# WestlyPark/StyleRenderer

Hardware: AMD Instinct MI355X
Metric: generator fwd+bwd images/sec at 256^2 (higher is better)
Workload: dtype f32

## Files before the change

include/stylerenderer_amd.h:

```cpp
#ifndef STYLERENDERER_AMD_H_
#define STYLERENDERER_AMD_H_

#include <stddef.h>
#include <stdint.h>

#ifdef __cplusplus
extern "C" {
#endif

typedef void* sr_stream_t;

#define SR_OK 0
#define SR_EINVAL (-1)
#define SR_ERANGE (-2)

const char* sr_error_string(int code);
int sr_abi_version(void);

int sr_fused_bias_act(float* y, const float* x, const float* b, const float* ref, int act, int grad,
                      float alpha, float scale, int64_t size_x, int64_t step_b, int64_t size_b,
                      int use_bias, int use_ref, sr_stream_t stream);

int64_t sr_fused_act_bwd_scratch_floats(int64_t n, int64_t c, int64_t inner);
int sr_fused_act_bwd(float* gx, float* gb, const float* gy, const float* out, float alpha,
// ... 246 lines not shown
#define SR_CONV_PATH_S2_BF16 2
#define SR_CONV_PATH_S2_WINO 3
#define SR_CONV_PATH_GEMM1X1 4
#define SR_CONV_PATH_CONVT_TAPS 5
#define SR_CONV_PATH_CONVT_BF16 6
#define SR_CONV_PATH_CONVT_FUSED_KS 7
#define SR_CONV_PATH_CONVT_FUSED 8
#define SR_CONV_PATH_CONVT_WINO 9
#define SR_CONV_PATH_STRIPS 0x100
int sr_conv2d_path(int64_t B, int64_t C, int64_t N, int64_t IH, int64_t IW, int64_t OH, int64_t OW, int ksize, int stride,
                   int pad, int transposed, const float* in, const float* out, const float* wt, int64_t wt_ld,
                   int have_scratch);
int64_t sr_conv2d_path_floats(int64_t B, int64_t C, int64_t N, int64_t IH, int64_t IW, int64_t OH, int64_t OW, int ksize,
                              int stride, int pad, int transposed, const float* in, const float* out, const float* wt,
                              int64_t wt_ld, int have_scratch);

int sr_conv2d_generic(float* y, const float* x, const float* w, const float* bias, int64_t B, int64_t C, int64_t N,
                      int64_t IH, int64_t IW, int64_t OH, int64_t OW, int kh, int kw, int sy, int sx, int py, int px,
                      sr_stream_t stream);
int sr_conv2d_generic_dgrad(float* dx, const float* g, const float* w, int64_t B, int64_t C, int64_t N, int64_t IH,
                            int64_t IW, int64_t OH, int64_t OW, int kh, int kw, int sy, int sx, int py, int px,
                            sr_stream_t stream);
int sr_conv2d_generic_wgrad(float* dw, const float* x, const float* g, int64_t B, int64_t C, int64_t N, int64_t IH,
                            int64_t IW, int64_t OH, int64_t OW, int kh, int kw, int sy, int sx, int py, int px,
                            sr_stream_t stream);
int sr_conv2d_mfma_ex(float* out, const float* in, const float* wt, const float* iscale,
                      const float* oscale, const float* obias, int64_t B, int64_t C, int64_t N,
                      int64_t wt_ld, int64_t IH, int64_t IW, int64_t OH, int64_t OW, int ksize,
                      int stride, int pad, int transposed, int flags, float* scratch, sr_stream_t stream);
int sr_conv1x1_add_supported(int64_t B, int64_t C, int64_t N, int64_t wt_ld, int64_t P, const float* in, const float* wt,
                             const float* out, const float* addend);
int sr_conv1x1_add(float* out, const float* in, const float* wt, const float* oscale, const float* addend, int64_t B,
                   int64_t C, int64_t N, int64_t wt_ld, int64_t P, sr_stream_t stream);
int sr_conv2d_nba_ex(float* out, const float* in, const float* wt, const float* iscale, const float* oscale,
                     const float* noise, const float* noise_w, const float* abias, float alpha, float gain,
                     int64_t B, int64_t C, int64_t N, int64_t wt_ld, int64_t H, int64_t W, int64_t noise_bstride,
                     int flags, float* scratch, sr_stream_t stream);

int64_t sr_conv2d_wgrad_scratch_floats(int64_t B, int64_t C, int64_t N, int64_t IH, int64_t IW,
                                       int64_t OH, int64_t OW, int ksize, int stride, int pad,
                                       int transposed);
int sr_conv2d_wgrad_mfma(float* dwt, const float* x, const float* gy, const float* xscale,
                         const float* gscale, int64_t B, int64_t C, int64_t N, int64_t IH,
                         int64_t IW, int64_t OH, int64_t OW, int ksize, int stride, int pad,
                         int transposed, float* scratch, sr_stream_t stream);
#define SR_WGRAD_PATH_INVALID (-1)
#define SR_WGRAD_PATH_DIRECT 0
#define SR_WGRAD_PATH_SMALL3 1
#define SR_WGRAD_PATH_WINO 2
#define SR_WGRAD_PATH_BF16_1X1 3
#define SR_WGRAD_PATH_BF16_S2 4
#define SR_WGRAD_PATH_S2_DMA 5
#define SR_WGRAD_PATH_S2_WINO 6
int sr_conv2d_wgrad_path(int64_t B, int64_t C, int64_t N, int64_t IH, int64_t IW, int64_t OH, int64_t OW, int ksize,
                         int stride, int pad, int transposed, const float* x, const float* gy);
int64_t sr_conv2d_wgrad_path_floats(int64_t B, int64_t C, int64_t N, int64_t IH, int64_t IW, int64_t OH, int64_t OW,
                                    int ksize, int stride, int pad, int transposed, const float* x, const float* gy);
int64_t sr_conv2d_wgrad_style_floats(int64_t B, int64_t C, int64_t N, int64_t IH, int64_t IW, int64_t OH, int64_t OW,
                                     int ksize, int stride, int pad, int transposed, const float* x, const float* gy);
int sr_conv2d_wgrad_style(float* dwt, float* gis, const float* x, const float* gy, const float* iscale,
                          const float* gscale, const float* wt, int64_t ldw, int64_t B, int64_t C, int64_t N, int64_t IH,
                          int64_t IW, int64_t OH, int64_t OW, int ksize, int stride, int pad, int transposed,
                          float* scratch, float* part, sr_stream_t stream);

int sr_signal_bump(uint32_t* counter, sr_stream_t stream);
int sr_signal_set(uint32_t* word, const uint32_t* epoch, sr_stream_t stream);
// ... 150 lines not shown
```

stylerenderer_amd/_lib.py:

```python
import ctypes
import os

_HERE = os.path.dirname(os.path.abspath(__file__))
LIB_PATH = os.environ.get("STYLERENDERER_AMD_LIB") or os.path.join(_HERE, "libstylerenderer_hip.so")

_i = ctypes.c_int
_l = ctypes.c_int64
_f = ctypes.c_float
_d = ctypes.c_double
_p = ctypes.c_void_p

SIGNATURES = {
    "sr_error_string": (ctypes.c_char_p, [_i]),
    "sr_abi_version": (_i, []),
    "sr_fused_bias_act": (_i, [_p, _p, _p, _p, _i, _i, _f, _f, _l, _l, _l, _i, _i, _p]),
    "sr_fused_act_bwd_scratch_floats": (_l, [_l, _l, _l]),
    "sr_fused_act_bwd": (_i, [_p, _p, _p, _p, _f, _f, _l, _l, _l, _p, _p]),
    "sr_noise_bias_act": (_i, [_p] * 6 + [_f, _f] + [_l] * 4 + [_p]),
    "sr_noise_bias_act_bwd_scratch_floats": (_l, [_l, _l, _l]),
    "sr_noise_bias_act_bwd": (_i, [_p] * 6 + [_f, _f] + [_l] * 4 + [_p, _p]),
    "sr_noise_bias_act_bwd_dot_scratch_floats": (_l, [_l, _l, _l]),
    "sr_noise_bias_act_bwd_dot": (_i, [_p] * 9 + [_f, _f] + [_l] * 4 + [_p, _p]),
    "sr_conv2d_nba": (_i, [_p] * 8 + [_f, _f] + [_l] * 7 + [_p, _p]),
    "sr_conv2d_nba_ex": (_i, [_p] * 8 + [_f, _f] + [_l] * 7 + [_i, _p, _p]),
# ... 64 lines not shown
    "sr_conv2d_generic_dgrad": (_i, [_p] * 3 + [_l] * 7 + [_i] * 6 + [_p]),
    "sr_conv2d_generic_wgrad": (_i, [_p] * 3 + [_l] * 7 + [_i] * 6 + [_p]),
    "sr_blur_nba_bwd_scratch_floats": (_l, [_l, _l, _i, _i]),
    "sr_blur_nba_bwd": (_i, [_p] * 10 + [_f, _f, _l, _l] + [_i] * 5 + [_l, _p, _p]),
    "sr_rasterize_scratch_bytes": (_l, [_l, _l, _l, _l, _i]),
    "sr_rasterize_grad_state_ints": (_l, [_l, _l]),
    "sr_rasterize_forward_f32": (_i, [_l] * 5 + [_i] * 3 + [_p] * 5 + [_f, _p, _l, _p, _p, _p, _p, _p]),
    "sr_rasterize_levels_supported": (_i, [_i, _l, _l, _p, _p]),
    "sr_rasterize_forward_levels_f32": (_i, [_i, _l, _l, _l, _p, _p, _i, _i, _i, _p, _p, _f, _p, _l, _p, _p, _p, _p, _p]),
    "sr_rasterize_grad_levels_f32": (_i, [_i, _l, _l, _l, _p, _p, _i, _i, _p, _p, _l] + [_p] * 6 + [_l, _l] + [_p] * 3 + [_f, _p, _p]),
    "sr_rasterize_forward_f64": (_i, [_l] * 5 + [_i] * 3 + [_p] * 5 + [_d, _p, _l, _p, _p, _p, _p, _p]),
    "sr_rasterize_grad_scratch_bytes": (_l, [_l, _l, _l, _i]),
    "sr_rasterize_forward_cpu_f32": (_i, [_l] * 5 + [_i] * 3 + [_p] * 5 + [_f]),
    "sr_rasterize_forward_cpu_f64": (_i, [_l] * 5 + [_i] * 3 + [_p] * 5 + [_d]),
    "sr_rasterize_backward_cpu_f32": (_i, [_l] * 4 + [_i] + [_p] * 3 + [_f]),
    "sr_rasterize_backward_cpu_f64": (_i, [_l] * 4 + [_i] + [_p] * 3 + [_d]),
    "sr_rasterize_backward_f32": (_i, [_l] * 4 + [_i] * 2 + [_p] * 3 + [_f, _p]),
    "sr_rasterize_backward_f64": (_i, [_l] * 4 + [_i] * 2 + [_p] * 3 + [_d, _p]),
    "sr_rasterize_grad_f32": (_i, [_l] * 5 + [_i] * 2 + [_p, _p, _l] + [_p] * 6 + [_l, _l, _p, _p, _p, _f, _p, _p]),
    "sr_conv2d_wgrad_scratch_floats": (_l, [_l] * 7 + [_i] * 4),
    "sr_conv2d_wgrad_mfma": (_i, [_p] * 5 + [_l] * 7 + [_i] * 4 + [_p, _p]),
    "sr_conv2d_scratch_floats": (_l, [_l] * 7 + [_i] * 4),
    "sr_conv2d_mfma": (_i, [_p] * 6 + [_l] * 8 + [_i] * 4 + [_p, _p]),
    "sr_conv2d_uses_winograd": (_i, [_l] * 5 + [_p, _p]),
    "sr_conv2d_path": (_i, [_l] * 7 + [_i] * 4 + [_p, _p, _p, _l, _i]),
    "sr_conv2d_path_floats": (_l, [_l] * 7 + [_i] * 4 + [_p, _p, _p, _l, _i]),
    "sr_conv2d_wgrad_path": (_i, [_l] * 7 + [_i] * 4 + [_p, _p]),
    "sr_conv2d_wgrad_path_floats": (_l, [_l] * 7 + [_i] * 4 + [_p, _p]),
    "sr_conv2d_wgrad_style_floats": (_l, [_l] * 7 + [_i] * 4 + [_p, _p]),
    "sr_conv2d_wgrad_style": (_i, [_p] * 7 + [_l] * 8 + [_i] * 4 + [_p, _p, _p]),
    "sr_conv2d_mfma_ex": (_i, [_p] * 6 + [_l] * 8 + [_i] * 5 + [_p, _p]),
    "sr_conv1x1_add_supported": (_i, [_l] * 5 + [_p] * 4),
    "sr_conv1x1_add": (_i, [_p] * 5 + [_l] * 5 + [_p]),
    "sr_rasterize_grad_f64": (_i, [_l] * 5 + [_i] * 2 + [_p, _p, _l] + [_p] * 6 + [_l, _l, _p, _p, _p, _d, _p, _p]),
    "sr_pose_fwd": (_i, [_p, _p, _p, _p]),
    "sr_pose_bwd": (_i, [_p, _p, _p, _p, _p]),
    "sr_pose_batch_fwd": (_i, [_p, _p, _p, _l, _p]),
    "sr_affine3_fwd": (_i, [_p, _p, _p, _p, _l, _l, _l, _p]),
    "sr_affine3_bwd": (_i, [_p, _p, _p, _p, _l, _l, _l, _p]),
    "sr_morph_fwd": (_i, [_p] * 9 + [_f, _l, _l, _l, _p]),
    "sr_vertex_normals_bwd_f32": (_i, [_p] * 11 + [_l, _l, _l, _f, _p]),
    "sr_morph_gcoeff_scratch_floats": (_l, [_l, _l, _l]),
    "sr_morph_gcoeff": (_i, [_p] * 6 + [_f, _p, _l, _l, _l, _p]),
    "sr_morph_pose_bwd": (_i, [_p] * 5 + [_l, _p]),
    "sr_skin_joints_fwd": (_i, [_p] * 11 + [_f] + [_l] * 4 + [_p]),
    "sr_skin_fwd": (_i, [_p] * 7 + [_l] * 4 + [_p]),
    "sr_skin_bwd_scratch_floats": (_l, [_l, _l, _l]),
    "sr_skin_bwd": (_i, [_p] * 7 + [_l] * 3 + [_p]),
    "sr_skin_joints_bwd": (_i, [_p] * 11 + [_f, _p] + [_l] * 5 + [_p]),
    "sr_blend_z_floats": (_l, [_l, _l, _l]),
    "sr_blend_head": (_i, [_p] * 6 + [_f] + [_l] * 3 + [_p]),
    "sr_blend_fwd": (_i, [_p] * 8 + [_l] * 4 + [_p]),
    "sr_blend_gz": (_i, [_p] * 3 + [_l] * 4 + [_p]),
    "sr_blend_tail": (_i, [_p] * 5 + [_f, _p] + [_l] * 3 + [_p]),
    "sr_resample_u8_scratch_bytes": (_l, [_l] * 6 + [ctypes.POINTER(ctypes.c_int32)] + [_l] * 4),
    "sr_resample_u8": (_i, [_p, _p] + [_l] * 6 + [_p, _p, ctypes.POINTER(ctypes.c_int32), _l] * 2 + [_l] * 4
                       + [_i, _i, _p, _p]),
    "sr_warp_affine_u8": (_i, [_p, _p, _p] + [_l] * 7 + [_i, _i, _i, _p]),
    "sr_landmark_loss_fwd": (_i, [_p] * 8 + [_l] * 5 + [_f, _f, _p]),
    "sr_landmark_loss_bwd": (_i, [_p, _p, _p, _l, _p, _p, _p] + [_l] * 5 + [_i, _p]),
    "sr_landmark_dyn_fwd": (_i, [_p] * 15 + [_l] * 6 + [_i, _f, _f, _l, _l, _f, _f, _p]),
    "sr_landmark_dyn_bwd": (_i, [_p, _p, _p, _l] + [_p] * 7 + [_l] * 6 + [_i, _p]),
    "sr_region_fill": (_i, [_p, _p, _p] + [_l] * 6 + [_p]),
    "sr_region_grow": (_i, [_p, _p, _l, _l, _l, _i, _p]),
    "sr_region_blend_fwd": (_i, [_p] * 6 + [_l] * 4 + [_f] + [_l] * 4 + [_p]),
    "sr_region_blend_bwd": (_i, [_p] * 3 + [_l] * 4 + [_p]),
# ... 85 lines not shown
```

stylerenderer_amd/build.py:

```python
import os
import subprocess
import sys

HERE = os.path.dirname(os.path.abspath(__file__))
CSRC = os.path.join(HERE, "csrc")
LIB = os.path.join(HERE, "libstylerenderer_hip.so")
OBJ = os.path.join(HERE, "csrc", "_obj")

ARCH = "gfx950"
COMMON = ["--offload-arch=" + ARCH, "-O3", "-std=c++17", "-fPIC", "-Wno-unused-result",
          "-fhip-fp32-correctly-rounded-divide-sqrt"]
EXACT = ["-ffp-contract=off"]
NOSLP = ["-fno-slp-vectorize"]

SOURCES = [
    ("capi.hip", EXACT),
    ("fused_bias_act.hip", EXACT),
    ("upfirdn2d.hip", EXACT + NOSLP),
    ("rasterize.hip", EXACT),
    ("rasterize_keys.hip", EXACT),
    ("rasterize_tiled.hip", EXACT),
    ("rasterize_grad.hip", EXACT),
    ("fused_elem.hip", EXACT),
    ("weight_prep.hip", EXACT),
# ... 3 lines not shown
    ("landmark.hip", EXACT),
    ("region.hip", EXACT),
    ("texture.hip", EXACT),
    ("texture_sample.hip", EXACT),
    ("texture_mip.hip", EXACT),
    ("share.hip", EXACT),
    ("camera.hip", EXACT),
    ("light.hip", EXACT),
    ("morph.hip", []),
    ("skin.hip", []),
    ("blend.hip", []),
    ("lpips.hip", EXACT),
    ("ppl.hip", EXACT),
    ("augment.hip", EXACT),
    ("resample.hip", EXACT),
    ("warp.hip", EXACT),
    ("conv_dispatch.hip", []),
    ("conv_mfma.hip", []),
    ("convt_fused.hip", []),
    ("conv_wino.hip", []),
    ("conv_wgrad_wino.hip", []),
    ("conv_wgrad_dispatch.hip", []),
    ("conv_wgrad_mfma.hip", []),
    ("conv_wgrad_s2_dma.hip", []),
    ("conv_wgrad_small3.hip", []),
    ("conv_wgrad_reduce.hip", []),
    ("conv_wgrad_bf16x3.hip", []),
    ("conv_wgrad_s2_wino.hip", []),
    ("conv_s2_bf16x3.hip", []),
    ("conv_s2_wino.hip", []),
    ("convt_wino.hip", []),
    ("conv_generic.hip", []),
    ("conv1x1_gemm.hip", []),
    ("inception.hip", []),
]


def _hipcc():
    for c in (os.environ.get("HIPCC"), "/opt/rocm/bin/hipcc", "hipcc"):
        if c and (os.path.isabs(c) and os.path.exists(c) or not os.path.isabs(c)):
            return c
    return "hipcc"


def _deps(src):
    deps = [src, os.path.join(CSRC, "common.h"),
            os.path.join(HERE, "..", "include", "stylerenderer_amd.h"), os.path.abspath(__file__)]
    deps += [os.path.join(CSRC, f) for f in os.listdir(CSRC) if f.endswith(".h")]
    return max(os.path.getmtime(d) for d in deps if os.path.exists(d))


def build_library(force=False, verbose=False):
    os.makedirs(OBJ, exist_ok=True)
    hipcc = _hipcc()
    objs, rebuilt = [], False
    procs = []
    for name, extra in SOURCES:
        src = os.path.join(CSRC, name)
        obj = os.path.join(OBJ, name.replace(".hip", ".o"))
        objs.append(obj)
        if force or not os.path.exists(obj) or os.path.getmtime(obj) < _deps(src):
            cmd = [hipcc] + COMMON + extra + ["-c", src, "-o", obj]
            if verbose:
                print(" ".join(cmd))
            procs.append((name, subprocess.Popen(cmd, stdout=subprocess.PIPE, stderr=subprocess.STDOUT)))
            rebuilt = True
# ... 18 lines not shown
```

stylerenderer_amd/csrc/conv_mfma.hip:

```cpp
#include "conv_mfma.h"

#include "conv1x1_gemm.h"
#include "mfma_tile.h"

#include <algorithm>
#include <cstdlib>

namespace {

constexpr int BN = 128;
constexpr int BM = 128;

__device__ __attribute__((aligned(16))) const float g_zero_line[4] = {0.f, 0.f, 0.f, 0.f};
__device__ __attribute__((aligned(16))) const float g_ones_line[4] = {1.f, 1.f, 1.f, 1.f};

template <int IS, int TY, int TX, int PW, int PH, int PB, bool V4, bool TAP9 = false>
struct Geo {
    static constexpr bool ROT = V4 && IS == 2;
    static constexpr int NT = TY * TX;
    static constexpr int KC = NT >= 9 ? 4 : (NT >= 4 ? 8 : 16);
    static constexpr int EH = (PH - 1) * IS + TY;
    static constexpr int EW = (PW - 1) * IS + TX;
    static constexpr int LEAD = (V4 && !ROT) ? (TAP9 ? 4 : (TX > 1 ? 3 : 0)) : 0;
    static constexpr int EWP = ROT ? (EW + 3 + 3) / 4 * 4
                                   : (V4 ? (LEAD + EW + 3) / 4 * 4 : EW + ((EW % 2 == 0) ? 1 : 0));
    static constexpr int PLANE = PB * EH * EWP;
    static constexpr int W_FLOATS = NT * KC * BN;
    static constexpr int W_INSTR = W_FLOATS / 256;
    static constexpr int IMG_INSTR = V4 ? (KC * PLANE + 255) / 256 : 0;
    static constexpr int ST_INSTR = V4 ? (KC * PB + 63) / 64 : 0;
    static constexpr int IN_FLOATS = KC * PLANE + KC * PB;
    static constexpr int IN_INSTR = V4 ? IMG_INSTR + ST_INSTR : (IN_FLOATS + 63) / 64;
    static constexpr int S_BASE = V4 ? W_FLOATS + IMG_INSTR * 256 : W_FLOATS + KC * PLANE;
    static constexpr int BUF = V4 ? S_BASE + ST_INSTR * 64 : W_FLOATS + IN_INSTR * 64;
    static constexpr int W_PER_WAVE = (W_INSTR + 3) / 4;
// ... 521 lines not shown
    p.GH = p.IH + 1; p.GW = p.IW + 1;
    p.gy_base = p.gx_base = 0;
    p.osy = p.osx = 2; p.ooy = p.oox = 0;
    p.dy0 = p.dx0 = 0;
    p.tap_first = 0; p.tap_step = 1; p.tap_count = 9;
    p.ks = ks; p.c_per_slice = c_per_slice;
    int pw, ph, pb;
    patch_shape(p.GW, pw, ph, pb);
    p.tiles_x = (p.GW + pw - 1) / pw;
    p.tiles_y = (p.GH + ph - 1) / ph;
    p.tiles_b = (p.B + pb - 1) / pb;
    p.tiles_n = (p.N + BN - 1) / BN;
    const int64_t blocks = (int64_t)p.tiles_x * p.tiles_y * p.tiles_b * p.tiles_n * p.ks * 9;
    if (blocks > 0x7FFFFFFFLL) return SR_ERANGE;
    const dim3 grid((unsigned)blocks);
    const bool v4 = taps_v4(p);
    int rc;
    if (gemm)
        rc = sr_convt_taps_gemm_launch(p.partial, p.in, p.wt, p.ldw, p.iscale, p.B, p.C, p.N, p.IH, p.IW, p.ks, p.c_per_slice, st);
    else if (pw == 32) rc = v4 ? launch_one<1, 1, 1, 32, 4, 1, true, true>(p, grid, st)
                          : launch_one<1, 1, 1, 32, 4, 1, false, true>(p, grid, st);
    else if (pw == 16) rc = v4 ? launch_one<1, 1, 1, 16, 8, 1, true, true>(p, grid, st)
                               : launch_one<1, 1, 1, 16, 8, 1, false, true>(p, grid, st);
    else if (pw == 8) rc = launch_one<1, 1, 1, 8, 8, 2, false, true>(p, grid, st);
    else rc = launch_one<1, 1, 1, 4, 4, 8, false, true>(p, grid, st);
    if (rc != SR_OK) return rc;
    const int64_t total = (int64_t)p.B * p.N * p.OH * p.OW;
    hipLaunchKernelGGL(k_convt_tap_reduce, dim3(sr_stream_grid(total, 256)), dim3(256), 0, st, p);
    return sr_launch_status();
}

int64_t sr_convt_strip_floats(int64_t B, int64_t N, int64_t IH, int64_t IW) { return STRIP_KS * 3 * B * N * (IW + 1 + IH); }

int sr_convt_strips_launch(ConvParams p, hipStream_t st) {
    float* prow = p.partial;
    float* pcol = p.partial + STRIP_KS * 3 * (int64_t)p.B * p.N * (p.IW + 1);
    p.osy = p.osx = 2; p.ooy = p.oox = 0;
    p.dy0 = p.dx0 = 0;
    p.ks = 1; p.c_per_slice = (p.C + 15) / 16 * 16;
    p.gy_base = p.IH; p.GH = p.IH + 1; p.gx_base = 0; p.GW = p.IW + 1;
    p.tap_first = 6; p.tap_step = 1; p.tap_count = 3;
    p.partial = prow;
    int rc = launch_strip_part<32, 4, 1>(p, st);
    if (rc != SR_OK) return rc;
    const int ks_row = p.ks;
    p.gy_base = 0; p.GH = p.IH; p.gx_base = p.IW; p.GW = p.IW + 1;
    p.tap_first = 2; p.tap_step = 3; p.tap_count = 3;
    p.partial = pcol;
    rc = launch_strip_part<4, 4, 8>(p, st);
    if (rc != SR_OK) return rc;
    const int ks_col = p.ks;
    const int64_t total = (int64_t)p.B * p.N * (p.OW + p.OH - 1);
    hipLaunchKernelGGL(k_convt_strip_reduce, dim3(sr_stream_grid(total, 256)), dim3(256), 0, st, p, prow, pcol, ks_row,
                       ks_col);
    return sr_launch_status();
}

int sr_convt_phases_launch(ConvParams p, bool interior_done, hipStream_t st) {
    for (int py = 0; py < 2; ++py)
        for (int px = 0; px < 2; ++px) {
            const int TYp = py == 0 ? 2 : 1, TXp = px == 0 ? 2 : 1;
            p.osy = p.osx = 2; p.ooy = py; p.oox = px;
            p.dy0 = -(TYp - 1); p.dx0 = -(TXp - 1);
            for (int ty = 0; ty < TYp; ++ty)
                for (int tx = 0; tx < TXp; ++tx) {
                    const int ky = py + 2 * (TYp - 1 - ty), kx = px + 2 * (TXp - 1 - tx);
                    p.wmap[ty * TXp + tx] = ky * 3 + kx;
// ... 26 lines not shown
```

stylerenderer_amd/csrc/upfirdn2d.hip:

```cpp
#include "common.h"

#include <cstdlib>
#include <type_traits>

namespace {

struct UfdParams {
    int in_h, in_w, out_h, out_w, kh, kw;
    int up_x, up_y, down_x, down_y, pad_x0, pad_y0;
};

__device__ __forceinline__ int floor_div(int a, int b) {
    int q = a / b;
    return (a % b != 0 && ((a < 0) != (b < 0))) ? q - 1 : q;
}

__global__ __launch_bounds__(256) void k_upfirdn_generic(float* __restrict__ out,
                                                         const float* __restrict__ x,
                                                         const float* __restrict__ k, UfdParams p,
                                                         int64_t total) {
    extern __shared__ float s_k[];
    for (int i = threadIdx.x; i < p.kh * p.kw; i += blockDim.x) {
        const int ky = i / p.kw, kx = i % p.kw;
        s_k[i] = k[(p.kh - 1 - ky) * p.kw + (p.kw - 1 - kx)];
// ... 560 lines not shown
#pragma unroll
            for (int kx = 0; kx < 4; ++kx) {
                const float prod = s_band[(er + ky) * ld + 4 + in_w - 2 + kx] * kf[ky * 4 + kx];
                edge = edge + prod;
            }
    }
    __syncthreads();
    const int64_t a0 = (plane * out_h + r0) * (int64_t)out_w;
    const int res = (int)(a0 & 3);
    if (active) {
#pragma unroll
        for (int r = 0; r < B_RPL; ++r) {
            if (ly + r >= rb) continue;
#pragma unroll
            for (int c = 0; c < 4; ++c) s_band[res + (ly + r) * out_w + ox + c] = acc[r][c];
        }
    }
    if (er >= 0) s_band[res + er * out_w + in_w] = edge;
    __syncthreads();
    const int end = res + rb * out_w;
    float* dst = out + (a0 - res);
    for (int j = 4 * (int)threadIdx.x; j < end; j += 4 * 256) {
        const float4 v = *reinterpret_cast<const float4*>(s_band + j);
        if (j >= res && j + 3 < end) {
            *reinterpret_cast<float4*>(dst + j) = v;
        } else {
            if (j >= res && j < end) dst[j] = v.x;
            if (j + 1 >= res && j + 1 < end) dst[j + 1] = v.y;
            if (j + 2 >= res && j + 2 < end) dst[j + 2] = v.z;
            if (j + 3 >= res && j + 3 < end) dst[j + 3] = v.w;
        }
    }
}

constexpr int R_OH = 32, R_OW = 32;

template <int UP, int DOWN>
__global__ __launch_bounds__(256) void k_fir4_resample(float* __restrict__ out, const float* __restrict__ x,
                                                       const float* __restrict__ k, int in_h, int in_w,
                                                       int out_h, int out_w, int pad_x0, int pad_y0,
                                                       int tiles_x, int tiles_y,
                                                       const float* __restrict__ addend) {
    static_assert((UP == 1 && DOWN == 2) || (UP == 2 && DOWN == 1), "one of the two resampling shapes");
    constexpr int SPAN_H = ((R_OH - 1) * DOWN + 4 + UP - 1) / UP + 1;
    constexpr int SPAN_W = ((R_OW - 1) * DOWN + 4 + UP - 1) / UP + 1;
    constexpr int LDW = SPAN_W | 1;
    __shared__ float s_in[SPAN_H * LDW];
    __shared__ float s_k[16];
    int bid = blockIdx.x;
    const int tx_i = bid % tiles_x;
    bid /= tiles_x;
    const int ty_i = bid % tiles_y;
    const int64_t plane = bid / tiles_y;
    const int oy0 = ty_i * R_OH, ox0 = tx_i * R_OW;
    const int my0 = oy0 * DOWN - pad_y0, mx0 = ox0 * DOWN - pad_x0;
    const int iy_lo = floor_div(my0 + UP - 1, UP), ix_lo = floor_div(mx0 + UP - 1, UP);
    const float* src = x + plane * (int64_t)in_h * in_w;
    if (threadIdx.x < 16) {
        const int ky = threadIdx.x >> 2, kx = threadIdx.x & 3;
        s_k[threadIdx.x] = k[(3 - ky) * 4 + (3 - kx)];
    }
    for (int i = threadIdx.x; i < SPAN_H * SPAN_W; i += 256) {
        const int r = i / SPAN_W, c = i - r * SPAN_W;
        const int gy = iy_lo + r, gx = ix_lo + c;
        const bool ok = gy >= 0 && gy < in_h && gx >= 0 && gx < in_w;
        s_in[r * LDW + c] = ok ? src[(int64_t)gy * in_w + gx] : 0.0f;
// ... 162 lines not shown
    if (in_h * 2 + pad0 + pad1 - 4 + 1 != out_h || in_w * 2 + pad0 + pad1 - 4 + 1 != out_w) return SR_EINVAL;
    if (major == 0 || out_h <= 0 || out_w <= 0) return SR_OK;
    if (!out || !x || !k || !addend) return SR_EINVAL;
    const int tiles_x = (out_w + R_OW - 1) / R_OW, tiles_y = (out_h + R_OH - 1) / R_OH;
    const int64_t blocks = (int64_t)tiles_x * tiles_y * major;
    if (blocks >= 0x7FFFFFFFLL) return SR_ERANGE;
    hipLaunchKernelGGL((k_fir4_resample<2, 1>), dim3((unsigned)blocks), dim3(256), 0, sr_stream(stream), out, x, k, in_h,
                       in_w, out_h, out_w, pad0, pad0, tiles_x, tiles_y, addend);
    return sr_launch_status();
}

extern "C" int sr_blur_noise_bias_act(float* y, const float* x, const float* k, const float* noise,
                                      const float* noise_w, const float* bias, float alpha, float gain, int64_t n,
                                      int64_t c, int in_h, int in_w, int out_h, int out_w, int pad0, int pad1,
                                      int64_t noise_bstride, sr_stream_t stream) {
    if (n < 0 || c < 0 || in_h < 0 || in_w < 0) return SR_EINVAL;
    if (in_h + pad0 + pad1 - 4 + 1 != out_h || in_w + pad0 + pad1 - 4 + 1 != out_w) return SR_EINVAL;
    if (n * c == 0 || out_h <= 0 || out_w <= 0) return SR_OK;
    if (!y || !x || !k || (noise && !noise_w)) return SR_EINVAL;
    const int tiles_x = (out_w + T_OW - 1) / T_OW, tiles_y = (out_h + T_OH - 1) / T_OH;
    const int64_t blocks = (int64_t)tiles_x * tiles_y * n * c;
    if (blocks >= 0x7FFFFFFFLL) return SR_ERANGE;
    const FirNba nba{noise, noise_w, bias, noise_bstride, (int)c, alpha, gain};
    if (fir4_band_enabled() && pad0 == 1 && pad1 == 1 && al16(x) && al16(y) &&
        (!noise || (al16(noise) && noise_bstride % 4 == 0))) {
        const FirBand g = fir4_band_geom(out_w, out_h);
        if (g.bands > 0 && (int64_t)g.bands * n * c < 0x7FFFFFFFLL && (int64_t)in_h * in_w < (1 << 30)) {
            const size_t lds = ((size_t)(g.rmax + 3) * in_w + 16) * sizeof(float);
            hipLaunchKernelGGL(k_fir4_band_fwd, dim3((unsigned)(g.bands * n * c)), dim3(256), lds, sr_stream(stream), y, x,
                               k, in_h, in_w, g.lanes_x, g.bands, n * c * (int64_t)in_h * in_w, nba);
            return sr_launch_status();
        }
    }
    if (fir4_aligned(x, in_w, pad0))
        hipLaunchKernelGGL((k_fir4_tile<true, true>), dim3((unsigned)blocks), dim3(256), 0, sr_stream(stream), y, x, k,
                           in_h, in_w, out_h, out_w, pad0, pad0, tiles_x, tiles_y, nba);
    else
        hipLaunchKernelGGL((k_fir4_tile<true, false>), dim3((unsigned)blocks), dim3(256), 0, sr_stream(stream), y, x, k,
                           in_h, in_w, out_h, out_w, pad0, pad0, tiles_x, tiles_y, nba);
    return sr_launch_status();
}

int sr_nba_finish_launch(float* gbias, float* gnoise_w, float* rowdot, const float* partial, const float* dot_partial,
                         float* chan_nw, int64_t n, int64_t c, int chunks, bool has_noise, hipStream_t st);

extern "C" int64_t sr_blur_nba_bwd_scratch_floats(int64_t n, int64_t c, int out_h, int out_w) {
    if (n <= 0 || c <= 0 || out_h <= 0 || out_w <= 0) return 3;
    const int64_t tiles = (int64_t)((out_w + T_OW - 1) / T_OW) * ((out_h + T_OH - 1) / T_OH);
    const int64_t bands = fir4_band_geom(out_w - 1, out_h).bands;
    return 3 * n * c * (tiles > bands ? tiles : bands) + c + 2;
}

extern "C" int sr_blur_nba_bwd(float* gx, float* gbias, float* gnoise_w, float* rowdot, const float* gy, const float* y,
                               const float* k_flipped, const float* noise, const float* noise_w, const float* bias,
                               float alpha, float gain, int64_t n, int64_t c, int in_h, int in_w, int out_h, int out_w,
                               int pad0, int64_t noise_bstride, float* scratch, sr_stream_t stream) {
    if (n < 0 || c < 0 || in_h < 0 || in_w < 0) return SR_EINVAL;
    if (out_h + 2 * pad0 - 3 != in_h || out_w + 2 * pad0 - 3 != in_w || pad0 < 0 || pad0 > 3) return SR_EINVAL;
    if (n * c == 0 || in_h == 0 || in_w == 0) return SR_OK;
    if (!gx || !rowdot || !gy || !y || !k_flipped || !scratch || (noise && !noise_w) || gain == 0.0f || alpha == 0.0f)
        return SR_EINVAL;
    const int tiles_x = (out_w + T_OW - 1) / T_OW, tiles_y = (out_h + T_OH - 1) / T_OH;
    const int gpad = 3 - pad0;
    const bool vec = al16(gy) && al16(y) && (!noise || (al16(noise) && noise_bstride % 4 == 0));
    FirBand band{0, 0, 0};
    if (fir4_band_enabled() && pad0 == 1 && vec && al16(gx)) band = fir4_band_geom(in_w, out_h);
    const int chunks = band.bands > 0 ? band.bands : tiles_x * tiles_y;
    const int64_t blocks = (int64_t)chunks * n * c;
    if (blocks >= 0x7FFFFFFFLL) return SR_ERANGE;
    if (tiles_y * T_OH - gpad < in_h || tiles_x * T_OW - gpad < in_w) return SR_EINVAL;
    hipStream_t st = sr_stream(stream);
    float* dot_partial = scratch + 2 * n * c * (int64_t)chunks;
    float* chan_nw = dot_partial + n * c * (int64_t)chunks;
    const FirNbaBwd q{y, noise, noise_w, bias, scratch, chunks == 1 ? rowdot : dot_partial, noise_bstride, (int)c, alpha,
                      gain, 1.0f / gain, 1.0f / (alpha * gain)};
    const bool aln = fir4_aligned(gy, in_w, gpad) && vec;
    if (band.bands > 0)
        hipLaunchKernelGGL(k_fir4_band_nba_bwd, dim3((unsigned)blocks), dim3(256),
                           (size_t)(band.rmax + 3) * (in_w + 8) * sizeof(float), st, gx, gy, k_flipped, in_h, in_w,
                           band.lanes_x, band.bands, q);
    else if (aln)
        hipLaunchKernelGGL(k_fir4_nba_bwd<true>, dim3((unsigned)blocks), dim3(256), 0, st, gx, gy, k_flipped, in_h, in_w,
                           out_h, out_w, gpad, gpad, tiles_x, tiles_y, q);
    else
        hipLaunchKernelGGL(k_fir4_nba_bwd<false>, dim3((unsigned)blocks), dim3(256), 0, st, gx, gy, k_flipped, in_h, in_w,
                           out_h, out_w, gpad, gpad, tiles_x, tiles_y, q);
    const int rc = sr_launch_status();
    if (rc != SR_OK) return rc;
    return sr_nba_finish_launch(gbias, gnoise_w, chunks == 1 ? nullptr : rowdot, scratch, dot_partial, chan_nw, n, c,
                                chunks, noise != nullptr, st);
}
```

Before: 637.0.

## Add MFMA border kernel for transposed conv and packed small-plane FIR kernels

Adds a new MFMA-based kernel that computes the border row and column of stride-2 transposed convolutions in one launch, replacing the strip-partial launches when the batch times border size is large enough. It also adds packed upfirdn kernels that process several small 8/16/32-wide planes per workgroup in LDS for both the forward and the noise-bias-act backward pass, replacing per-tile launches that leave most threads idle on small planes. Both paths are enabled by default above size thresholds and can be switched off through environment variables. They add code complexity, and the border kernel's cross-wave LDS reduction and the packed kernel's edge handling are new places where correctness can break.

```diff
diff --git a/include/stylerenderer_amd.h b/include/stylerenderer_amd.h
--- a/include/stylerenderer_amd.h
+++ b/include/stylerenderer_amd.h
@@ -302,6 +302,9 @@
                              const float* out, const float* addend);
 int sr_conv1x1_add(float* out, const float* in, const float* wt, const float* oscale, const float* addend, int64_t B,
                    int64_t C, int64_t N, int64_t wt_ld, int64_t P, sr_stream_t stream);
+int sr_convt_border(float* out, const float* in, const float* wt, const float* iscale, const float* oscale,
+                    const float* obias, int64_t B, int64_t C, int64_t N, int64_t wt_ld, int64_t IH, int64_t IW,
+                    sr_stream_t stream);
 int sr_conv2d_nba_ex(float* out, const float* in, const float* wt, const float* iscale, const float* oscale,
                      const float* noise, const float* noise_w, const float* abias, float alpha, float gain,
                      int64_t B, int64_t C, int64_t N, int64_t wt_ld, int64_t H, int64_t W, int64_t noise_bstride,
diff --git a/stylerenderer_amd/_lib.py b/stylerenderer_amd/_lib.py
--- a/stylerenderer_amd/_lib.py
+++ b/stylerenderer_amd/_lib.py
@@ -120,6 +120,7 @@
     "sr_conv2d_mfma_ex": (_i, [_p] * 6 + [_l] * 8 + [_i] * 5 + [_p, _p]),
     "sr_conv1x1_add_supported": (_i, [_l] * 5 + [_p] * 4),
     "sr_conv1x1_add": (_i, [_p] * 5 + [_l] * 5 + [_p]),
+    "sr_convt_border": (_i, [_p] * 6 + [_l] * 6 + [_p]),
     "sr_rasterize_grad_f64": (_i, [_l] * 5 + [_i] * 2 + [_p, _p, _l] + [_p] * 6 + [_l, _l, _p, _p, _p, _d, _p, _p]),
     "sr_pose_fwd": (_i, [_p, _p, _p, _p]),
     "sr_pose_bwd": (_i, [_p, _p, _p, _p, _p]),
diff --git a/stylerenderer_amd/build.py b/stylerenderer_amd/build.py
--- a/stylerenderer_amd/build.py
+++ b/stylerenderer_amd/build.py
@@ -59,6 +59,7 @@
     ("convt_wino.hip", []),
     ("conv_generic.hip", []),
     ("conv1x1_gemm.hip", []),
+    ("convt_border.hip", []),
     ("inception.hip", []),
 ]
 
diff --git a/stylerenderer_amd/csrc/conv_mfma.hip b/stylerenderer_amd/csrc/conv_mfma.hip
--- a/stylerenderer_amd/csrc/conv_mfma.hip
+++ b/stylerenderer_amd/csrc/conv_mfma.hip
@@ -1,6 +1,7 @@
 #include "conv_mfma.h"
 
 #include "conv1x1_gemm.h"
+#include "convt_border.h"
 #include "mfma_tile.h"
 
 #include <algorithm>
@@ -588,7 +589,16 @@
 
 int64_t sr_convt_strip_floats(int64_t B, int64_t N, int64_t IH, int64_t IW) { return STRIP_KS * 3 * B * N * (IW + 1 + IH); }
 
+constexpr int64_t CONVT_BORDER_MIN_POINTS = 1024;
+static_assert(CONVT_BORDER_MIN_POINTS > 8 * (32 + 32 + 1), "the t3s2 row of tests/conv_plan_cases.py stays on the strip launches");
+static_assert(CONVT_BORDER_MIN_POINTS <= 4 * (128 + 128 + 1), "batch 4's 128^2 up-sampling layer takes k_convt_border");
+
 int sr_convt_strips_launch(ConvParams p, hipStream_t st) {
+    {
+        const int sw = sr_env_char("SR_CONVT_BORDER");
+        const int64_t points = (int64_t)p.B * (p.IH + p.IW + 1);
+        if (sw != '0' && (sw == 'f' || points >= CONVT_BORDER_MIN_POINTS)) return sr_convt_border_launch(p, st);
+    }
     float* prow = p.partial;
     float* pcol = p.partial + STRIP_KS * 3 * (int64_t)p.B * p.N * (p.IW + 1);
     p.osy = p.osx = 2; p.ooy = p.oox = 0;
diff --git a/stylerenderer_amd/csrc/convt_border.h b/stylerenderer_amd/csrc/convt_border.h
--- /dev/null
+++ b/stylerenderer_amd/csrc/convt_border.h
@@ -0,0 +1,7 @@
+#pragma once
+#include <hip/hip_runtime.h>
+#include <stdint.h>
+
+#include "conv_params.h"
+
+int sr_convt_border_launch(const ConvParams& p, hipStream_t st);
diff --git a/stylerenderer_amd/csrc/convt_border.hip b/stylerenderer_amd/csrc/convt_border.hip
--- /dev/null
+++ b/stylerenderer_amd/csrc/convt_border.hip
@@ -0,0 +1,249 @@
+#include "mfma_tile.h"
+#include "convt_border.h"
+
+namespace {
+
+constexpr int BT_N = 64, BT_P = 64, BKC = 8;
+constexpr int BKS = BKC / 2;
+
+struct BorderParams {
+    const float* in;
+    const float* wt;
+    const float* iscale;
+    const float* oscale;
+    const float* obias;
+    float* out;
+    int B, C, N, ldw, IH, IW, OH, OW;
+    int tiles_n;
+    int row_tiles;
+};
+
+struct Chunk {
+    float wa[BKS][2], wb[BKS][2], wo[BKS][2], x[BKS][2], xe[BKS][2], s[BKS][2];
+};
+
+template <bool ISC>
+__global__ __launch_bounds__(256, 1) void k_convt_border(const BorderParams q) {
+#if __HIP_DEVICE_COMPILE__
+    __shared__ float s_red[4][3][16][64];
+    int bid = blockIdx.x;
+    const int tn = bid % q.tiles_n;
+    int tq = bid / q.tiles_n;
+    const bool is_row = tq < q.row_tiles;
+    if (!is_row) tq -= q.row_tiles;
+    const int tap_a = is_row ? 6 : 2, tap_o = is_row ? 7 : 5, tap_b = 8;
+    const int pps = is_row ? q.IW + 1 : q.IH;
+    const int64_t total = (int64_t)q.B * pps;
+    const int n0 = tn * BT_N;
+    const int tid = threadIdx.x, lane = tid & 63, wave = tid >> 6;
+    const int l31 = lane & 31, half = lane >> 5;
+    const int plane = q.IH * q.IW;
+
+    bool okp[2], ok_a[2], ok_b[2];
+    int bq[2], opos[2];
+    const float* xa[2];
+    const float* xe[2];
+#pragma unroll
+    for (int j = 0; j < 2; ++j) {
+        const int64_t q0 = (int64_t)tq * BT_P + j * 32, qi = q0 + l31;
+        okp[j] = qi < total;
+        bq[j] = okp[j] ? (int)(qi / pps) : 0;
+        const int g = okp[j] ? (int)(qi - (int64_t)bq[j] * pps) : 0;
+        ok_a[j] = okp[j] && (!is_row || g < q.IW);
+        ok_b[j] = okp[j] && g >= 1;
+        const int pos_a = is_row ? (q.IH - 1) * q.IW + (g < q.IW ? g : q.IW - 1) : g * q.IW + q.IW - 1;
+        xa[j] = q.in + ((int64_t)bq[j] * q.C + half) * plane + pos_a;
+        opos[j] = is_row ? (q.OH - 1) * q.OW + 2 * g : 2 * g * q.OW + q.OW - 1;
+        const bool ok0 = q0 < total;
+        const int b0 = ok0 ? (int)(q0 / pps) : 0;
+        const int g0 = ok0 ? (int)(q0 - (int64_t)b0 * pps) : 0;
+        const int pos_e = g0 >= 1 ? (is_row ? (q.IH - 1) * q.IW + g0 - 1 : (g0 - 1) * q.IW + q.IW - 1) : 0;
+        xe[j] = q.in + ((int64_t)b0 * q.C + half) * plane + pos_e;
+    }
+    const int ostep = is_row ? 1 : q.OW;
+    bool okn[2];
+    int ncol[2];
+#pragma unroll
+    for (int i = 0; i < 2; ++i) {
+        const int n = n0 + i * 32 + l31;
+        okn[i] = n < q.N;
+        ncol[i] = okn[i] ? n : q.N - 1;
+    }
+
+    const int nch = (q.C + BKC - 1) / BKC;
+    const int per = (nch + 3) / 4;
+    const int ch_beg = min(wave * per, nch), ch_end = min(ch_beg + per, nch);
+    const int64_t tap_stride = (int64_t)q.C * q.ldw;
+
+    auto fetch = [&](int ch, Chunk& r) {
+        const int c0 = ch * BKC + half;
+#pragma unroll
+        for (int kk = 0; kk < BKS; ++kk) {
+            const int c = min(c0 + 2 * kk, q.C - 1);
+            const int64_t dc = (int64_t)(c - half) * plane;
+            const float* wr = q.wt + (int64_t)c * q.ldw;
+#pragma unroll
+            for (int i = 0; i < 2; ++i) {
+                r.wa[kk][i] = wr[tap_a * tap_stride + ncol[i]];
+                r.wb[kk][i] = wr[tap_b * tap_stride + ncol[i]];
+                r.wo[kk][i] = wr[tap_o * tap_stride + ncol[i]];
+            }
+#pragma unroll
+            for (int j = 0; j < 2; ++j) {
+                r.x[kk][j] = xa[j][dc];
+                r.xe[kk][j] = xe[j][dc];
+                r.s[kk][j] = ISC ? q.iscale[(int64_t)bq[j] * q.C + c] : 1.0f;
+            }
+        }
+    };
+
+    f32x16 acc[2][2][2];
+#pragma unroll
+    for (int e = 0; e < 2; ++e)
+#pragma unroll
+        for (int i = 0; i < 2; ++i)
+#pragma unroll
+            for (int j = 0; j < 2; ++j)
+#pragma unroll
+                for (int r = 0; r < 16; ++r) acc[e][i][j][r] = 0.0f;
+
+    auto mma = [&](int ch, const Chunk& r) {
+        const int c0 = ch * BKC + half;
+#pragma unroll
+        for (int kk = 0; kk < BKS; ++kk) {
+            const bool ck = c0 + 2 * kk < q.C;
+            float wa[2], wb[2], wo[2], xa_[2], xb_[2];
+#pragma unroll
+            for (int i = 0; i < 2; ++i) {
+                const bool m = ck & okn[i];
+                wa[i] = m ? r.wa[kk][i] : 0.0f;
+                wb[i] = m ? r.wb[kk][i] : 0.0f;
+                wo[i] = m ? r.wo[kk][i] : 0.0f;
+            }
+#pragma unroll
+            for (int j = 0; j < 2; ++j) {
+                const float left = __shfl_up(r.x[kk][j], 1, 32);
+                const float xb = l31 == 0 ? r.xe[kk][j] : left;
+                const float pa = r.x[kk][j] * r.s[kk][j], pb = xb * r.s[kk][j];
+                xa_[j] = (ck & ok_a[j]) ? pa : 0.0f;
+                xb_[j] = (ck & ok_b[j]) ? pb : 0.0f;
+            }
+#pragma unroll
+            for (int i = 0; i < 2; ++i)
+#pragma unroll
+                for (int j = 0; j < 2; ++j) {
+                    acc[0][i][j] = __builtin_amdgcn_mfma_f32_32x32x2f32(wa[i], xa_[j], acc[0][i][j], 0, 0, 0);
+                    acc[0][i][j] = __builtin_amdgcn_mfma_f32_32x32x2f32(wb[i], xb_[j], acc[0][i][j], 0, 0, 0);
+                    acc[1][i][j] = __builtin_amdgcn_mfma_f32_32x32x2f32(wo[i], xa_[j], acc[1][i][j], 0, 0, 0);
+                }
+        }
+    };
+
+    static_assert(sizeof(Chunk) / sizeof(float) < 63, "a chunk's loads are countable by s_waitcnt vmcnt");
+    Chunk r0, r1;
+    if (ch_beg < ch_end) {
+        fetch(ch_beg, r0);
+        int ch = ch_beg;
+        for (; ch + 2 < ch_end; ch += 2) {
+            fetch(ch + 1, r1);
+            __builtin_amdgcn_sched_barrier(0);
+            mma(ch, r0);
+            __builtin_amdgcn_sched_barrier(0);
+            fetch(ch + 2, r0);
+            __builtin_amdgcn_sched_barrier(0);
+            mma(ch + 1, r1);
+            __builtin_amdgcn_sched_barrier(0);
+        }
+        if (ch + 1 < ch_end) {
+            fetch(ch + 1, r1);
+            __builtin_amdgcn_sched_barrier(0);
+            mma(ch, r0);
+            mma(ch + 1, r1);
+        } else {
+            mma(ch, r0);
+        }
+    }
+
+    const int qi = wave >> 1, qj = wave & 1;
+    const bool okq = qj ? okp[1] : okp[0];
+    const bool okodd = qj ? ok_a[1] : ok_a[0];
+    const int b = qj ? bq[1] : bq[0];
+    const int64_t plane_out = (int64_t)q.OH * q.OW;
+    float* dst = q.out + (int64_t)b * q.N * plane_out + (qj ? opos[1] : opos[0]);
+#pragma unroll
+    for (int e = 0; e < 2; ++e) {
+        auto pass = [&](int quad, const f32x16& v) {
+            if (quad == wave) return;
+            const int slot = quad < wave ? quad : quad - 1;
+#pragma unroll
+            for (int r = 0; r < 16; ++r) s_red[wave][slot][r][lane] = v[r];
+        };
+        if (e) __syncthreads();
+        pass(0, acc[e][0][0]);
+        pass(1, acc[e][0][1]);
+        pass(2, acc[e][1][0]);
+        pass(3, acc[e][1][1]);
+        __syncthreads();
+        f32x16 sum;
+#pragma unroll
+        for (int v = 0; v < 4; ++v) {
+            if (v == wave) {
+                const f32x16 own = wave == 0 ? acc[e][0][0] : (wave == 1 ? acc[e][0][1] : (wave == 2 ? acc[e][1][0] : acc[e][1][1]));
+#pragma unroll
+                for (int r = 0; r < 16; ++r) sum[r] = v == 0 ? own[r] : sum[r] + own[r];
+            } else {
+                const int slot = wave < v ? wave : wave - 1;
+#pragma unroll
+                for (int r = 0; r < 16; ++r) sum[r] = v == 0 ? s_red[v][slot][r][lane] : sum[r] + s_red[v][slot][r][lane];
+            }
+        }
+        if (e ? okodd : okq) {
+            float* d = dst + e * ostep;
+#pragma unroll
+            for (int r = 0; r < 16; ++r) {
+                const int n = n0 + sr_mfma32_row(r, half, qi * 32);
+                if (n >= q.N) continue;
+                float v = sum[r];
+                if (q.oscale) v *= q.oscale[(int64_t)b * q.N + n];
+                if (q.obias) v += q.obias[n];
+                d[(int64_t)n * plane_out] = v;
+            }
+        }
+    }
+#endif
+}
+
+}
+
+int sr_convt_border_launch(const ConvParams& p, hipStream_t st) {
+    if (p.B <= 0 || p.C <= 0 || p.N <= 0 || p.IH <= 0 || p.IW <= 0 || p.OH != 2 * p.IH + 1 || p.OW != 2 * p.IW + 1 ||
+        p.ldw < p.N || !p.in || !p.wt || !p.out)
+        return SR_EINVAL;
+    if ((int64_t)p.IH * p.IW > 0x7FFFFFFF || (int64_t)p.OH * p.OW > 0x7FFFFFFF) return SR_ERANGE;
+    BorderParams q;
+    q.in = p.in; q.wt = p.wt; q.iscale = p.iscale; q.oscale = p.oscale; q.obias = p.obias; q.out = p.out;
+    q.B = p.B; q.C = p.C; q.N = p.N; q.ldw = p.ldw; q.IH = p.IH; q.IW = p.IW; q.OH = p.OH; q.OW = p.OW;
+    q.tiles_n = (p.N + BT_N - 1) / BT_N;
+    const int64_t row_tiles = sr_ceil_div((int64_t)p.B * (p.IW + 1), BT_P);
+    const int64_t blocks = (row_tiles + sr_ceil_div((int64_t)p.B * p.IH, BT_P)) * q.tiles_n;
+    if (blocks > 0x7FFFFFFFLL) return SR_ERANGE;
+    q.row_tiles = (int)row_tiles;
+    if (q.iscale) hipLaunchKernelGGL(k_convt_border<true>, dim3((unsigned)blocks), dim3(256), 0, st, q);
+    else hipLaunchKernelGGL(k_convt_border<false>, dim3((unsigned)blocks), dim3(256), 0, st, q);
+    return sr_launch_status();
+}
+
+extern "C" int sr_convt_border(float* out, const float* in, const float* wt, const float* iscale, const float* oscale,
+                               const float* obias, int64_t B, int64_t C, int64_t N, int64_t wt_ld, int64_t IH, int64_t IW,
+                               sr_stream_t stream) {
+    if (B < 0 || C <= 0 || N <= 0 || IH <= 0 || IW <= 0 || wt_ld < N) return SR_EINVAL;
+    if (B == 0) return SR_OK;
+    if (!out || !in || !wt) return SR_EINVAL;
+    if (B > 0x7FFFFFFF || C > 0x7FFFFFFF || N > 0x7FFFFFFF || wt_ld > 0x7FFFFFFF || IH > (1 << 29) || IW > (1 << 29))
+        return SR_ERANGE;
+    ConvParams p{};
+    p.in = in; p.wt = wt; p.iscale = iscale; p.oscale = oscale; p.obias = obias; p.out = out;
+    p.B = (int)B; p.C = (int)C; p.N = (int)N; p.ldw = (int)wt_ld; p.IH = (int)IH; p.IW = (int)IW;
+    p.OH = 2 * p.IH + 1; p.OW = 2 * p.IW + 1;
+    return sr_convt_border_launch(p, sr_stream(stream));
+}
diff --git a/stylerenderer_amd/csrc/upfirdn2d.hip b/stylerenderer_amd/csrc/upfirdn2d.hip
--- a/stylerenderer_amd/csrc/upfirdn2d.hip
+++ b/stylerenderer_amd/csrc/upfirdn2d.hip
@@ -616,6 +616,212 @@
         }
     }
 }
+
+constexpr int P_OUT = 2048;
+
+template <int S>
+struct FirPack {
+    static_assert(S == 8 || S == 16 || S == 32, "2^k sides below the band kernels' floor");
+    static constexpr int PP = P_OUT / (S * S);
+    static constexpr int LPP = S * S / 8;
+    static constexpr int LX = S / 4;
+    static constexpr int LD = S + 4;
+    static constexpr int PS_F = (S + 3) * LD;
+    static constexpr int PS_B = (S + 4) * LD;
+};
+
+template <int N>
+__device__ __forceinline__ void pack_zero_lds(float* s) {
+    static_assert(N % 4 == 0, "whole 16-byte groups");
+    for (int i = threadIdx.x; i < N / 4; i += 256) reinterpret_cast<float4*>(s)[i] = make_float4(0.f, 0.f, 0.f, 0.f);
+}
+
+template <int S>
+__global__ __launch_bounds__(256) void k_fir4_pack_fwd(float* __restrict__ out, const float* __restrict__ x,
+                                                       const float* __restrict__ k, int64_t planes, FirNba nba) {
+    using P = FirPack<S>;
+    constexpr int IN = S + 1, PE = IN * IN, NE = P::PP * PE, ST = (NE + 255) / 256;
+    __shared__ __attribute__((aligned(16))) float s_in[P::PP * P::PS_F];
+    const int64_t plane0 = (int64_t)blockIdx.x * P::PP;
+    const int64_t left = planes - plane0;
+    const int ne = left < P::PP ? (int)left * PE : NE;
+    const float* src = x + plane0 * PE;
+    FIR4_LOAD_TAPS(kf, k)
+
+    float stage[ST];
+#pragma unroll
+    for (int j = 0; j < ST; ++j) {
+        const int e = threadIdx.x + 256 * j;
+        stage[j] = src[e < ne ? e : 0];
+    }
+    pack_zero_lds<P::PP * P::PS_F>(s_in);
+    __syncthreads();
+#pragma unroll
+    for (int j = 0; j < ST; ++j) {
+        const int e = threadIdx.x + 256 * j;
+        const int pl = e / PE, rem = e - pl * PE;
+        const int r = rem / IN, c = rem - r * IN;
+        if (e < ne) s_in[pl * P::PS_F + (r + 1) * P::LD + c + 1] = stage[j];
+    }
+    __syncthreads();
+
+    const int pl = threadIdx.x / P::LPP, lt = threadIdx.x - pl * P::LPP;
+    const int64_t plane = plane0 + pl;
+    if (plane >= planes) return;
+    const int lx = (lt % P::LX) * 4, ly = (lt / P::LX) * 2;
+    float acc[2][4];
+    fir4_rows<P::LD, 0>(s_in + pl * P::PS_F, kf, lx, ly, acc);
+
+    const int64_t b = plane / nba.channels;
+    const float* nz = nba.noise ? nba.noise + b * nba.noise_bstride : nullptr;
+    const float nw = nz ? nba.noise_w[0] : 0.0f;
+    const float bb = nba.bias ? nba.bias[plane - b * nba.channels] : 0.0f;
+    float* dst = out + plane * (int64_t)(S * S);
+#pragma unroll
+    for (int r = 0; r < 2; ++r) {
+        const int o = (ly + r) * S + lx;
+        float nr[4] = {0.0f, 0.0f, 0.0f, 0.0f};
+        if (nz) {
+            const float4 v = *reinterpret_cast<const float4*>(nz + o);
+            nr[0] = v.x; nr[1] = v.y; nr[2] = v.z; nr[3] = v.w;
+        }
+#pragma unroll
+        for (int c = 0; c < 4; ++c) {
+            float v = acc[r][c];
+            if (nz) v = v + nw * nr[c];
+            v += bb;
+            acc[r][c] = ((v > 0.0f) ? v : v * nba.alpha) * nba.gain;
+        }
+        *reinterpret_cast<float4*>(dst + o) = make_float4(acc[r][0], acc[r][1], acc[r][2], acc[r][3]);
+    }
+}
+
+template <int S>
+__global__ __launch_bounds__(256) void k_fir4_pack_nba_bwd(float* __restrict__ out, const float* __restrict__ gy,
+                                                           const float* __restrict__ k, int64_t planes, FirNbaBwd q) {
+    using P = FirPack<S>;
+    constexpr int ON = S + 1, PE = ON * ON, NE = P::PP * PE;
+    constexpr int L = S * S / 4;
+    constexpr int LW = L < 64 ? L : 64;
+    static_assert(NE <= P::PP * P::PS_B, "the gradient span fits the staging tiles");
+    __shared__ __attribute__((aligned(16))) float s_in[P::PP * P::PS_B];
+    __shared__ float s_red[2][12];
+    const int64_t plane0 = (int64_t)blockIdx.x * P::PP;
+    FIR4_LOAD_TAPS(kf, k)
+
+    float4 sg[2], so[2], sn[2];
+    float nw[2], bb[2];
+    bool ok[2];
+#pragma unroll
+    for (int j = 0; j < 2; ++j) {
+        const int g = threadIdx.x + 256 * j;
+        const int pl = g / L;
+        const int64_t plane = plane0 + pl;
+        ok[j] = plane < planes;
+        const int64_t pc = ok[j] ? plane : planes - 1;
+        const int64_t b = pc / q.channels;
+        const int64_t o = pc * (int64_t)(S * S) + 4 * (g - pl * L);
+        sg[j] = *reinterpret_cast<const float4*>(gy + o);
+        so[j] = *reinterpret_cast<const float4*>(q.fw + o);
+        sn[j] = q.noise ? *reinterpret_cast<const float4*>(q.noise + b * q.noise_bstride + 4 * (g - pl * L))
+                        : make_float4(0.f, 0.f, 0.f, 0.f);
+        nw[j] = q.noise ? q.noise_w[0] : 0.0f;
+        bb[j] = q.bias ? q.bias[pc - b * q.channels] : 0.0f;
+    }
+    pack_zero_lds<P::PP * P::PS_B>(s_in);
+    __syncthreads();
+#pragma unroll
+    for (int j = 0; j < 2; ++j) {
+        const int g = threadIdx.x + 256 * j;
+        const int pl = g / L, e = 4 * (g - pl * L);
+        const int r = e / S, c = e - r * S;
+        FirSums s{0.0f, 0.0f, 0.0f};
+        float v[4];
+        v[0] = fir4_gpre(sg[j].x, so[j].x, sn[j].x, ok[j], ok[j], q, nw[j], bb[j], s);
+        v[1] = fir4_gpre(sg[j].y, so[j].y, sn[j].y, ok[j], ok[j], q, nw[j], bb[j], s);
+        v[2] = fir4_gpre(sg[j].z, so[j].z, sn[j].z, ok[j], ok[j], q, nw[j], bb[j], s);
+        v[3] = fir4_gpre(sg[j].w, so[j].w, sn[j].w, ok[j], ok[j], q, nw[j], bb[j], s);
+        float* d = s_in + pl * P::PS_B + (r + 2) * P::LD + c + 2;
+        *reinterpret_cast<float2*>(d) = make_float2(v[0], v[1]);
+        *reinterpret_cast<float2*>(d + 2) = make_float2(v[2], v[3]);
+#pragma unroll
+        for (int m = LW / 2; m > 0; m >>= 1) {
+            s.b += __shfl_xor(s.b, m, SR_WAVE);
+            s.n += __shfl_xor(s.n, m, SR_WAVE);
+            s.d += __shfl_xor(s.d, m, SR_WAVE);
+        }
+        if (L <= 64) {
+            if ((threadIdx.x & (LW - 1)) == 0 && ok[j]) {
+                const int64_t plane = plane0 + pl;
+                q.partial[plane * 2] = s.b;
+                q.partial[plane * 2 + 1] = s.n;
+                q.dot_partial[plane] = s.d;
+            }
+        } else {
+            const int lane = threadIdx.x & 63, wave = threadIdx.x >> 6;
+            if (lane == 0) { s_red[j][wave] = s.b; s_red[j][4 + wave] = s.n; s_red[j][8 + wave] = s.d; }
+        }
+    }
+    __syncthreads();
+    if (L > 64 && threadIdx.x < 2 && plane0 + threadIdx.x < planes) {
+        const float* r = s_red[threadIdx.x];
+        const int64_t plane = plane0 + threadIdx.x;
+        q.partial[plane * 2] = (r[0] + r[1]) + (r[2] + r[3]);
+        q.partial[plane * 2 + 1] = (r[4] + r[5]) + (r[6] + r[7]);
+        q.dot_partial[plane] = (r[8] + r[9]) + (r[10] + r[11]);
+    }
+
+    const int pl = threadIdx.x / P::LPP, lt = threadIdx.x - pl * P::LPP;
+    const int lx = (lt % P::LX) * 4, ly = (lt / P::LX) * 2;
+    const float* tile = s_in + pl * P::PS_B;
+    float acc[2][4];
+    fir4_rows<P::LD, 0>(tile, kf, lx, ly, acc);
+    constexpr int NEDGE = 2 * S + 1, ET = (NEDGE + P::LPP - 1) / P::LPP;
+    float edge[ET];
+#pragma unroll
+    for (int t = 0; t < ET; ++t) {
+        const int i = lt + t * P::LPP;
+        const int oy = i <= S ? i : S, ox = i <= S ? S : i - ON;
+        float a = 0.0f;
+        if (i < NEDGE) {
+#pragma unroll
+            for (int ky = 0; ky < 4; ++ky)
+#pragma unroll
+                for (int kx = 0; kx < 4; ++kx) {
+                    const float prod = tile[(oy + ky) * P::LD + ox + kx] * kf[ky * 4 + kx];
+                    a = a + prod;
+                }
+        }
+        edge[t] = a;
+    }
+    __syncthreads();
+    float* go = s_in + pl * PE;
+#pragma unroll
+    for (int r = 0; r < 2; ++r)
+#pragma unroll
+        for (int c = 0; c < 4; ++c) go[(ly + r) * ON + lx + c] = acc[r][c];
+#pragma unroll
+    for (int t = 0; t < ET; ++t) {
+        const int i = lt + t * P::LPP;
+        const int oy = i <= S ? i : S, ox = i <= S ? S : i - ON;
+        if (i < NEDGE) go[oy * ON + ox] = edge[t];
+    }
+    __syncthreads();
+    const int64_t left = planes - plane0;
+    const int ne = left < P::PP ? (int)left * PE : NE;
+    float* dst = out + plane0 * PE;
+    for (int e = threadIdx.x; e < ne; e += 256) dst[e] = s_in[e];
+}
+
+constexpr int64_t FIR_PACK_MIN_PLANES = 256;
+
+inline bool fir4_pack_wanted(int64_t planes) {
+    const int e = sr_env_char("SR_FIR_PACK");
+    if (e < 0 || e == '0') return false;
+    return e == 'f' || planes >= FIR_PACK_MIN_PLANES;
+}
+
+inline bool fir4_pack_side(int s) { return s == 8 || s == 16 || s == 32; }
 
 constexpr int R_OH = 32, R_OW = 32;
 
@@ -844,6 +1050,16 @@
             return sr_launch_status();
         }
     }
+    if (pad0 == 1 && pad1 == 1 && out_h == out_w && fir4_pack_side(out_w) && fir4_aligned_enabled() && al16(x) && al16(y) &&
+        (!noise || (al16(noise) && noise_bstride % 4 == 0)) && fir4_pack_wanted(n * c)) {
+        const int64_t planes = n * c;
+        const int64_t wgs = sr_ceil_div(planes * out_h * out_w, P_OUT);
+        hipStream_t st = sr_stream(stream);
+        if (out_w == 8) hipLaunchKernelGGL(k_fir4_pack_fwd<8>, dim3((unsigned)wgs), dim3(256), 0, st, y, x, k, planes, nba);
+        else if (out_w == 16) hipLaunchKernelGGL(k_fir4_pack_fwd<16>, dim3((unsigned)wgs), dim3(256), 0, st, y, x, k, planes, nba);
+        else hipLaunchKernelGGL(k_fir4_pack_fwd<32>, dim3((unsigned)wgs), dim3(256), 0, st, y, x, k, planes, nba);
+        return sr_launch_status();
+    }
     if (fir4_aligned(x, in_w, pad0))
         hipLaunchKernelGGL((k_fir4_tile<true, true>), dim3((unsigned)blocks), dim3(256), 0, sr_stream(stream), y, x, k,
                            in_h, in_w, out_h, out_w, pad0, pad0, tiles_x, tiles_y, nba);
@@ -877,7 +1093,9 @@
     const bool vec = al16(gy) && al16(y) && (!noise || (al16(noise) && noise_bstride % 4 == 0));
     FirBand band{0, 0, 0};
     if (fir4_band_enabled() && pad0 == 1 && vec && al16(gx)) band = fir4_band_geom(in_w, out_h);
-    const int chunks = band.bands > 0 ? band.bands : tiles_x * tiles_y;
+    const bool pack = band.bands == 0 && pad0 == 1 && in_h == in_w && fir4_pack_side(in_w) && fir4_aligned_enabled() && vec &&
+                      al16(gx) && fir4_pack_wanted(n * c);
+    const int chunks = band.bands > 0 ? band.bands : (pack ? 1 : tiles_x * tiles_y);
     const int64_t blocks = (int64_t)chunks * n * c;
     if (blocks >= 0x7FFFFFFFLL) return SR_ERANGE;
     if (tiles_y * T_OH - gpad < in_h || tiles_x * T_OW - gpad < in_w) return SR_EINVAL;
@@ -891,7 +1109,13 @@
         hipLaunchKernelGGL(k_fir4_band_nba_bwd, dim3((unsigned)blocks), dim3(256),
                            (size_t)(band.rmax + 3) * (in_w + 8) * sizeof(float), st, gx, gy, k_flipped, in_h, in_w,
                            band.lanes_x, band.bands, q);
-    else if (aln)
+    else if (pack) {
+        const int64_t planes = n * c;
+        const dim3 grid((unsigned)sr_ceil_div(planes * in_h * in_w, P_OUT));
+        if (in_w == 8) hipLaunchKernelGGL(k_fir4_pack_nba_bwd<8>, grid, dim3(256), 0, st, gx, gy, k_flipped, planes, q);
+        else if (in_w == 16) hipLaunchKernelGGL(k_fir4_pack_nba_bwd<16>, grid, dim3(256), 0, st, gx, gy, k_flipped, planes, q);
+        else hipLaunchKernelGGL(k_fir4_pack_nba_bwd<32>, grid, dim3(256), 0, st, gx, gy, k_flipped, planes, q);
+    } else if (aln)
         hipLaunchKernelGGL(k_fir4_nba_bwd<true>, dim3((unsigned)blocks), dim3(256), 0, st, gx, gy, k_flipped, in_h, in_w,
                            out_h, out_w, gpad, gpad, tiles_x, tiles_y, q);
     else
```

Result: no change. 640.2 (median of 6 runs) (+0.5%).
